# wolearyc/ramannoodle

Hardware: NVIDIA B200
Metric: md_frames_per_s (higher is better)
Workload: dtype f64

## Files before the change

include/ramannoodle_b200_debug.h:

```cpp
#ifndef RAMANNOODLE_B200_DEBUG_H
#define RAMANNOODLE_B200_DEBUG_H

#include "ramannoodle_b200.h"

#ifdef __cplusplus
extern "C" {
#endif

void rn_debug_force_generic_affine(int on);
void rn_debug_set_affine_config(int mt, int stages);
void rn_debug_set_dense_config(int version, int variant);
int64_t rn_debug_phase_tiles(int64_t num_frames, int64_t first_frame, int64_t stripe, int phase, int64_t* tiles,
                             int64_t capacity);
void rn_debug_set_dense_split(int mode);
void rn_debug_set_sweep_fused(int on);
void rn_debug_set_sweep_min_run(int run);
int rn_debug_fft_forward(rn_spectrum_plan* plan, const double* d_in, double* d_out, void* stream);
int rn_debug_fft_convolve(rn_spectrum_plan* plan, const double* d_in, double* d_out, void* stream);

#ifdef __cplusplus
}
#endif

#endif
```

ramannoodle_b200/_lib.py:

```python
from __future__ import annotations

import ctypes
import os

from .exceptions import NativeLibraryError

_HERE = os.path.dirname(os.path.abspath(__file__))
LIB_PATH = os.path.join(_HERE, "libramannoodle_b200.so")

c_double_p = ctypes.POINTER(ctypes.c_double)
c_int32_p = ctypes.POINTER(ctypes.c_int32)
c_int64_p = ctypes.POINTER(ctypes.c_int64)

RN_MODEL_DEFAULT = 0
RN_MODEL_FORCE_DENSE = 1

PROTOTYPES = {
    "rn_last_error": (ctypes.c_char_p, []),
    "rn_device_info": (ctypes.c_int, [ctypes.c_int] + [ctypes.POINTER(ctypes.c_int)] * 4),
    "rn_model_create": (ctypes.c_int, [ctypes.c_void_p, ctypes.c_int64, ctypes.c_void_p, ctypes.c_void_p,
                                       ctypes.c_int64, ctypes.c_void_p, ctypes.c_void_p, ctypes.c_void_p,
                                       ctypes.c_void_p, ctypes.c_void_p, ctypes.c_void_p, ctypes.c_void_p,
                                       ctypes.c_int, ctypes.c_int, ctypes.POINTER(ctypes.c_void_p)]),
    "rn_model_destroy": (ctypes.c_int, [ctypes.c_void_p]),
    "rn_model_info": (ctypes.c_int, [ctypes.c_void_p, c_int64_p]),
    "rn_calc_polarizabilities": (ctypes.c_int, [ctypes.c_void_p, ctypes.c_void_p, ctypes.c_int64,
                                                ctypes.c_void_p, ctypes.c_void_p]),
    "rn_get_polarizability": (ctypes.c_int, [ctypes.c_void_p, ctypes.c_void_p, ctypes.c_int64,
                                             ctypes.c_void_p, ctypes.c_void_p]),
    "rn_calc_polarizabilities_host": (ctypes.c_int, [ctypes.c_void_p, ctypes.c_void_p, ctypes.c_int64,
                                                     ctypes.c_void_p, ctypes.c_void_p, ctypes.c_int64]),
    "rn_calc_polarizabilities_multi": (ctypes.c_int, [ctypes.c_void_p, ctypes.c_void_p, ctypes.c_int64,
                                                      ctypes.c_void_p, ctypes.c_int, ctypes.c_void_p]),
    "rn_calc_polarizabilities_host_multi": (ctypes.c_int, [ctypes.c_void_p, ctypes.c_void_p, ctypes.c_int64,
                                                           ctypes.c_void_p, ctypes.c_int, ctypes.c_int64,
                                                           ctypes.c_void_p]),
    "rn_calc_polarizabilities_routed": (ctypes.c_int, [ctypes.c_void_p, ctypes.c_void_p, ctypes.c_int64,
                                                       ctypes.c_void_p, ctypes.c_void_p, ctypes.c_int, ctypes.c_int64,
                                                       ctypes.c_int64, ctypes.c_int64, ctypes.c_void_p]),
    "rn_routed_phases_supported": (ctypes.c_int, [ctypes.c_void_p, ctypes.c_void_p, ctypes.c_int64, ctypes.c_int64,
                                                  ctypes.c_int64]),
    "rn_calc_polarizabilities_routed_phase": (ctypes.c_int, [ctypes.c_void_p, ctypes.c_void_p, ctypes.c_int64,
                                                             ctypes.c_void_p, ctypes.c_void_p, ctypes.c_int,
                                                             ctypes.c_int64, ctypes.c_int64, ctypes.c_int64,
                                                             ctypes.c_int64, ctypes.c_int, ctypes.c_void_p]),
    "rn_calc_polarizabilities_host_routed": (ctypes.c_int, [ctypes.c_void_p, ctypes.c_void_p, ctypes.c_int64,
                                                            ctypes.c_void_p, ctypes.c_void_p, ctypes.c_int,
                                                            ctypes.c_int64, ctypes.c_int64, ctypes.c_int64,
                                                            ctypes.c_int64, ctypes.c_void_p]),
    "rn_apply_pbc": (ctypes.c_int, [ctypes.c_void_p, ctypes.c_void_p, ctypes.c_int64, ctypes.c_void_p]),
    "rn_spectrum_plan_create": (ctypes.c_int, [ctypes.c_int64, ctypes.c_int, ctypes.POINTER(ctypes.c_void_p)]),
    "rn_spectrum_plan_destroy": (ctypes.c_int, [ctypes.c_void_p]),
    "rn_spectrum_num_points": (ctypes.c_int64, [ctypes.c_int64]),
    "rn_md_spectrum": (ctypes.c_int, [ctypes.c_void_p, ctypes.c_void_p, ctypes.c_double, ctypes.c_int,
                                      ctypes.c_double, ctypes.c_int, ctypes.c_double, ctypes.c_void_p,
                                      ctypes.c_void_p, ctypes.c_void_p]),
    "rn_spectrum_plan_create_dist": (ctypes.c_int, [ctypes.c_int64, ctypes.c_int, ctypes.c_int, ctypes.c_int,
                                                    ctypes.POINTER(ctypes.c_void_p)]),
    "rn_spectrum_plan_info": (ctypes.c_int, [ctypes.c_void_p, c_int64_p]),
    "rn_spectrum_dist_sizes": (ctypes.c_int, [ctypes.c_void_p, c_int64_p, c_int64_p, c_int64_p]),
    "rn_spectrum_dist_route": (ctypes.c_int, [ctypes.c_void_p, c_int64_p, c_int64_p]),
    "rn_spectrum_dist_stripe": (ctypes.c_int, [ctypes.c_void_p, c_int64_p]),
    "rn_spectrum_dist_pack": (ctypes.c_int, [ctypes.c_void_p, ctypes.c_void_p, ctypes.c_void_p, ctypes.c_void_p,
                                             ctypes.c_int, ctypes.c_int, ctypes.c_int, ctypes.c_void_p]),
    "rn_spectrum_dist_transform": (ctypes.c_int, [ctypes.c_void_p, ctypes.c_void_p, ctypes.c_void_p, ctypes.c_int,
                                                  ctypes.c_void_p]),
    "rn_spectrum_dist_final": (ctypes.c_int, [ctypes.c_void_p, ctypes.c_void_p, ctypes.c_void_p, ctypes.c_void_p,
                                              ctypes.c_int, ctypes.c_double, ctypes.c_int, ctypes.c_double,
                                              ctypes.c_int, ctypes.c_double, ctypes.c_void_p, ctypes.c_void_p]),
    "rn_spectrum_dist_finish": (ctypes.c_int, [ctypes.c_void_p, ctypes.c_void_p, ctypes.c_double, ctypes.c_void_p,
                                               ctypes.c_void_p, ctypes.c_void_p]),
    "rn_signal_spectrum": (ctypes.c_int, [ctypes.c_void_p, ctypes.c_void_p, ctypes.c_double, ctypes.c_void_p,
                                          ctypes.c_void_p, ctypes.c_void_p]),
    "rn_convolve_workspace_size": (ctypes.c_size_t, [ctypes.c_int64, ctypes.c_int64]),
    "rn_convolve_spectrum": (ctypes.c_int, [ctypes.c_void_p, ctypes.c_void_p, ctypes.c_int64, ctypes.c_int,
                                            ctypes.c_double, ctypes.c_void_p, ctypes.c_int64, ctypes.c_void_p,
                                            ctypes.c_void_p, ctypes.c_void_p]),
    "rn_calc_polarizabilities_sweep": (ctypes.c_int, [ctypes.c_void_p, ctypes.c_int, ctypes.c_void_p, ctypes.c_int64,
                                                      ctypes.c_void_p, ctypes.c_void_p]),
    "rn_calc_polarizabilities_host_sweep": (ctypes.c_int, [ctypes.c_void_p, ctypes.c_int, ctypes.c_void_p,
                                                           ctypes.c_int64, ctypes.c_void_p, ctypes.c_int64]),
    "rn_calc_polarizabilities_sweep_routed": (ctypes.c_int, [ctypes.c_void_p, ctypes.c_int, ctypes.c_void_p,
                                                             ctypes.c_int64, ctypes.c_void_p, ctypes.c_void_p,
                                                             ctypes.c_int, ctypes.c_int64, ctypes.c_int64,
                                                             ctypes.c_int64, ctypes.c_void_p]),
    "rn_calc_polarizabilities_host_sweep_routed": (ctypes.c_int, [ctypes.c_void_p, ctypes.c_int, ctypes.c_void_p,
                                                                  ctypes.c_int64, ctypes.c_void_p, ctypes.c_void_p,
                                                                  ctypes.c_int, ctypes.c_int64, ctypes.c_int64,
                                                                  ctypes.c_int64, ctypes.c_int64, ctypes.c_void_p]),
    "rn_xdatcar_scan": (ctypes.c_int, [ctypes.c_char_p, c_int64_p, c_int64_p, ctypes.c_void_p]),
    "rn_xdatcar_read": (ctypes.c_int, [ctypes.c_char_p, ctypes.c_void_p, ctypes.c_int64, ctypes.c_int64,
                                       ctypes.c_int, ctypes.c_int]),
    "rn_outcar_scan": (ctypes.c_int, [ctypes.c_char_p, c_int64_p, c_int64_p, ctypes.c_void_p, ctypes.c_void_p]),
    "rn_outcar_read": (ctypes.c_int, [ctypes.c_char_p, ctypes.c_void_p, ctypes.c_int64, ctypes.c_int64,
                                      ctypes.c_void_p, ctypes.c_int, ctypes.c_int]),
    "rn_vasprun_scan": (ctypes.c_int, [ctypes.c_char_p, c_int64_p, c_int64_p, c_double_p]),
    "rn_vasprun_read": (ctypes.c_int, [ctypes.c_char_p, ctypes.c_void_p, ctypes.c_int64, ctypes.c_int64,
                                       ctypes.c_int, ctypes.c_int]),
    "rn_host_apply_pbc": (ctypes.c_int, [ctypes.c_void_p, ctypes.c_void_p, ctypes.c_int64, ctypes.c_int]),
    "rn_host_register": (ctypes.c_int, [ctypes.c_void_p, ctypes.c_size_t]),
    "rn_host_unregister": (ctypes.c_int, [ctypes.c_void_p]),
    "rn_bspline_to_pp": (ctypes.c_int, [ctypes.c_void_p, ctypes.c_int, ctypes.c_void_p, ctypes.c_int,
                                        ctypes.c_void_p, ctypes.c_void_p, ctypes.c_void_p]),
    "rn_launch_count": (ctypes.c_int64, []),
}

DEBUG_PROTOTYPES = {
    "rn_debug_force_generic_affine": (None, [ctypes.c_int]),
    "rn_debug_set_affine_config": (None, [ctypes.c_int, ctypes.c_int]),
    "rn_debug_set_dense_config": (None, [ctypes.c_int, ctypes.c_int]),
    "rn_debug_phase_tiles": (ctypes.c_int64, [ctypes.c_int64, ctypes.c_int64, ctypes.c_int64, ctypes.c_int, c_int64_p,
                                              ctypes.c_int64]),
    "rn_debug_set_dense_split": (None, [ctypes.c_int]),
    "rn_debug_set_sweep_fused": (None, [ctypes.c_int]),
    "rn_debug_set_sweep_min_run": (None, [ctypes.c_int]),
    "rn_debug_fft_forward": (ctypes.c_int, [ctypes.c_void_p, ctypes.c_void_p, ctypes.c_void_p, ctypes.c_void_p]),
    "rn_debug_fft_convolve": (ctypes.c_int, [ctypes.c_void_p, ctypes.c_void_p, ctypes.c_void_p, ctypes.c_void_p]),
}

_lib = None


def lib() -> ctypes.CDLL:
    global _lib
    if _lib is None:
        if not os.path.exists(LIB_PATH):
            raise NativeLibraryError(
                f"{LIB_PATH} not found — build it with `python -m ramannoodle_b200._build` "
                "(there is no CPU fallback)")
        try:
            handle = ctypes.CDLL(LIB_PATH)
        except OSError as exc:
            raise NativeLibraryError(f"cannot load {LIB_PATH}: {exc}") from exc
        for name, (restype, argtypes) in PROTOTYPES.items():
            try:
                fn = getattr(handle, name)
            except AttributeError as exc:
                raise NativeLibraryError(f"{LIB_PATH} does not export {name}") from exc
            fn.restype = restype
            fn.argtypes = argtypes
        for name, (restype, argtypes) in DEBUG_PROTOTYPES.items():
            fn = getattr(handle, name)
            fn.restype = restype
            fn.argtypes = argtypes
        _lib = handle
    return _lib


def last_error() -> str:
    return lib().rn_last_error().decode("utf-8", "replace")


def check(status: int, what: str) -> None:
    if status == 0:
        return
    message = last_error()
    if status == -1:
        raise ValueError(f"{what}: {message}")
    if status == -4:
        raise MemoryError(f"{what}: {message}")
    raise NativeLibraryError(f"{what} failed ({status}): {message}")


def require_device(device: int = 0) -> dict:
    rt = ctypes.c_int()
    count = ctypes.c_int()
    cc = ctypes.c_int()
    sms = ctypes.c_int()
    status = lib().rn_device_info(device, ctypes.byref(rt), ctypes.byref(count), ctypes.byref(cc), ctypes.byref(sms))
    if status != 0:
        raise NativeLibraryError(f"no usable CUDA device {device}: {last_error()} (there is no CPU fallback)")
    if cc.value // 10 != 10:
        raise NativeLibraryError(f"device {device} is sm_{cc.value}; ramannoodle_b200 is built for sm_100a only")
    return {"runtime": rt.value, "devices": count.value, "compute_capability": cc.value, "sm_count": sms.value}


def launch_count() -> int:
    return int(lib().rn_launch_count())
```

ramannoodle_b200/csrc/rn_device.cuh:

```cuda
#pragma once

#include "rn_common.cuh"

namespace rn {

struct Alpha0 {
    double v[9];
};

__device__ __forceinline__ double wrap_disp(double pos, double ref) {
    const double d = pos - ref;
    return d - ceil(d - 0.5);
}

__device__ __forceinline__ double wrap_disp_fast(double pos, double ref) {
    const double d = pos - ref;
    const unsigned mag = (unsigned)__double2hiint(d) & 0x7fffffffu;
    if (mag < 0x3fe00000u) return d;
    return d - ceil(d - 0.5);
}

__device__ __forceinline__ void dmma884(double& c0, double& c1, double a, double b) {
    asm("mma.sync.aligned.m8n8k4.row.col.f64.f64.f64.f64 {%0,%1}, {%2}, {%3}, {%0,%1};"
        : "+d"(c0), "+d"(c1)
        : "d"(a), "d"(b));
}

__device__ __forceinline__ uint32_t smem_u32(const void* p) { return (uint32_t)__cvta_generic_to_shared(p); }

__device__ __forceinline__ void cp_async_16(uint32_t dst, const void* src, int src_bytes) {
    asm volatile("cp.async.cg.shared.global [%0], [%1], 16, %2;" ::"r"(dst), "l"(src), "r"(src_bytes) : "memory");
}
__device__ __forceinline__ void cp_async_8(uint32_t dst, const void* src, int src_bytes) {
    asm volatile("cp.async.ca.shared.global [%0], [%1], 8, %2;" ::"r"(dst), "l"(src), "r"(src_bytes) : "memory");
}
__device__ __forceinline__ void cp_async_commit() { asm volatile("cp.async.commit_group;" ::: "memory"); }
template <int N>
__device__ __forceinline__ void cp_async_wait() {
    asm volatile("cp.async.wait_group %0;" ::"n"(N) : "memory");
}

__device__ __forceinline__ void mbar_init(uint32_t bar, uint32_t count) {
    asm volatile("mbarrier.init.shared::cta.b64 [%0], %1;" ::"r"(bar), "r"(count) : "memory");
}
__device__ __forceinline__ void mbar_arrive_expect_tx(uint32_t bar, uint32_t bytes) {
    asm volatile("mbarrier.arrive.expect_tx.shared::cta.b64 _, [%0], %1;" ::"r"(bar), "r"(bytes) : "memory");
}
__device__ __forceinline__ void mbar_wait(uint32_t bar, uint32_t parity) {
    asm volatile(
        "{\n"
        ".reg .pred p;\n"
        "WAIT_%=:\n"
        "mbarrier.try_wait.parity.shared::cta.b64 p, [%0], %1;\n"
        "@p bra DONE_%=;\n"
        "bra WAIT_%=;\n"
        "DONE_%=:\n"
        "}\n" ::"r"(bar),
        "r"(parity)
        : "memory");
}
__device__ __forceinline__ void tma_bulk_g2s(uint32_t dst, const void* src, uint32_t bytes, uint32_t bar) {
    asm volatile("cp.async.bulk.shared::cluster.global.mbarrier::complete_tx::bytes [%0], [%1], %2, [%3];" ::"r"(dst),
                 "l"(src), "r"(bytes), "r"(bar)
                 : "memory");
}

}
```

ramannoodle_b200/csrc/rn_polarizability.cu:

```cuda
#include "rn_device.cuh"

namespace rn {

template <bool WRAP>
__global__ void __launch_bounds__(256) affine_generic_kernel(const double* __restrict__ in,
                                                             const double* __restrict__ ref,
                                                             const double* __restrict__ G, int64_t frame_begin,
                                                             int64_t frame_end, int K, Alpha0 a0,
                                                             double* __restrict__ alpha) {
    const int lane = threadIdx.x & 31;
    const int g = lane >> 2, t = lane & 3;
    const int64_t warps = (int64_t)gridDim.x * (blockDim.x >> 5);
    const int64_t groups = (frame_end - frame_begin + 7) / 8;
    for (int64_t grp = (int64_t)blockIdx.x * (blockDim.x >> 5) + (threadIdx.x >> 5); grp < groups; grp += warps) {
        const int64_t frame = frame_begin + grp * 8 + g;
        const bool valid = frame < frame_end;
        const double* row = in + (valid ? frame : frame_begin) * (int64_t)K;
        double c0 = 0, c1 = 0, d0 = 0, d1 = 0;
        for (int e0 = 0; e0 < K; e0 += 4) {
            const int e = e0 + t;
            double a = 0, b = 0, b2 = 0;
            if (e < K) {
                if (valid) {
                    a = __ldg(row + e);
// ... 64 lines not shown

    if (threadIdx.x == 0) {
        for (int s = 0; s < STAGES; s++) mbar_init(full0 + 8 * s, 1);
        asm volatile("fence.mbarrier_init.release.cluster;" ::: "memory");
        asm volatile("fence.proxy.async;" ::: "memory");
        for (int s = 0; s < STAGES; s++) {
            const int64_t tile = blockIdx.x + (int64_t)s * gridDim.x;
            if (tile < num_tiles) issue_tile(tile, s);
        }
    }
    for (int e = threadIdx.x; e < slack; e += blockDim.x) {
        tab_ref[e] = WRAP ? __ldg(ref + e) : 0.0;
        tab_g9[e] = __ldg(G + (int64_t)e * 9 + 8);
    }
    __syncthreads();

    const int g = lane >> 2, t = lane & 3;
    const int kbase = warp * 8 * KP + 2 * t;
    double b8[KP][2];
    uint32_t validmask = 0;
#pragma unroll
    for (int p = 0; p < KP; p++) {
#pragma unroll
        for (int h = 0; h < 2; h++) {
            const int e = kbase + 8 * p + h;
            b8[p][h] = __ldg(G + (int64_t)e * 9 + g);
            if (e < K) validmask |= 1u << (2 * p + h);
        }
    }
    const double* my_ref = tab_ref + kbase;
    const double* my_g9 = tab_g9 + kbase;
    const int rowoff = g * row_stride + kbase;
    double* myred = red + ((size_t)warp * ROWS + g) * kRedStride;

    int64_t i = 0;
    int64_t pending_row0 = -1;
    TileCursor here, ahead;
    if (SELECT) {
        cursor_set(sel, blockIdx.x, here);
        cursor_set(sel, blockIdx.x + (int64_t)STAGES * gridDim.x, ahead);
    }
    for (int64_t tile = blockIdx.x; tile < num_tiles; tile += gridDim.x, i++) {
        const int s = (int)(i % STAGES);
        const int64_t tile_row0 = (SELECT ? cursor_tile(sel, here) : tile) * ROWS;
        const bool stage_rows = peers_bulk && (tile_row0 + ROWS <= num_frames);
        mbar_wait(full0 + 8 * s, (uint32_t)(i / STAGES) & 1);
        const double* base = stages + (size_t)s * stage_doubles + rowoff;
        double c0[MT][2], c1[MT][2], a9[MT][2];
#pragma unroll
        for (int m = 0; m < MT; m++)
#pragma unroll
            for (int h = 0; h < 2; h++) c0[m][h] = c1[m][h] = a9[m][h] = 0.0;
#pragma unroll
        for (int p = 0; p < KP; p++) {
            const double2 g9 = *reinterpret_cast<const double2*>(my_g9 + 8 * p);
            double2 rf = make_double2(0.0, 0.0);
            if (WRAP) rf = *reinterpret_cast<const double2*>(my_ref + 8 * p);
#pragma unroll
            for (int m = 0; m < MT; m++) {
                const double2 v = *reinterpret_cast<const double2*>(base + (size_t)m * 8 * row_stride + 8 * p);
                double a_lo = v.x, a_hi = v.y;
                if (WRAP) {
                    a_lo = wrap_disp(a_lo, rf.x);
                    a_hi = wrap_disp(a_hi, rf.y);
                }
                a_lo = (validmask >> (2 * p)) & 1u ? a_lo : 0.0;
                a_hi = (validmask >> (2 * p + 1)) & 1u ? a_hi : 0.0;
                dmma884(c0[m][0], c1[m][0], a_lo, b8[p][0]);
                a9[m][0] = fma(a_lo, g9.x, a9[m][0]);
                dmma884(c0[m][1], c1[m][1], a_hi, b8[p][1]);
                a9[m][1] = fma(a_hi, g9.y, a9[m][1]);
            }
        }
        double* slot = myred + (size_t)(i & 1) * RED;
#pragma unroll
        for (int m = 0; m < MT; m++) {
            double a9s = a9[m][0] + a9[m][1];
            a9s += __shfl_xor_sync(0xffffffffu, a9s, 1);
            a9s += __shfl_xor_sync(0xffffffffu, a9s, 2);
            *reinterpret_cast<double2*>(slot + (size_t)m * 8 * kRedStride + 2 * t) =
                make_double2(c0[m][0] + c0[m][1], c1[m][0] + c1[m][1]);
            if (t == 0) slot[(size_t)m * 8 * kRedStride + 8] = a9s;
        }
        __syncthreads();
        if (peers_bulk && threadIdx.x == 32 && pending_row0 >= 0) {
            const uint32_t src = smem_u32(outbuf + (size_t)((i - 1) & 1) * ROWS * 9);
            const uint32_t mask = alpha_peer_mask(peers, pending_row0, ROWS);
            const int64_t off = alpha_peer_offset(peers, pending_row0);
            for (int p = 0; p < peers.count; p++)
                if (((mask >> p) & 1u) && peers.ptr[p])
                    asm volatile("cp.async.bulk.global.shared::cta.bulk_group [%0], [%1], %2;" ::"l"(peers.ptr[p] + off),
                                 "r"(src), "r"((uint32_t)(ROWS * 72))
                                 : "memory");
            asm volatile("cp.async.bulk.commit_group;" ::: "memory");
        }
        {
            const int64_t next = tile + (int64_t)STAGES * gridDim.x;
            if (next < num_tiles && lane == 0) {
                const int64_t frame0 = (SELECT ? cursor_tile(sel, ahead) : next) * ROWS;
                const int rows = (int)min((int64_t)ROWS, num_frames - frame0);
                if (warp == 0) mbar_arrive_expect_tx(full0 + 8 * s, row_bytes * rows);
                const uint32_t dst0 = smem_u32(stages + (size_t)s * stage_doubles);
                const double* src0 = in + frame0 * (int64_t)K;
                for (int r = warp; r < rows; r += kAffineWarps)
                    tma_bulk_g2s(dst0 + (uint32_t)(r * row_stride) * 8u, src0 + (int64_t)r * K, row_bytes,
                                 full0 + 8 * s);
            }
        }
        if (threadIdx.x < 9 * ROWS) {
            const int f = threadIdx.x / 9, q = threadIdx.x % 9;
            const double* r = red + (size_t)(i & 1) * RED + (size_t)f * kRedStride + q;
            double sum = 0;
#pragma unroll
            for (int w = 0; w < kAffineWarps; w++) sum += r[(size_t)w * ROWS * kRedStride];
            const int64_t frame = tile_row0 + f;
            const double value = sum + a0.v[q];
            if (frame < num_frames) alpha[frame * 9 + q] = value;
            if (stage_rows) {
                outbuf[(size_t)(i & 1) * ROWS * 9 + threadIdx.x] = value;
                asm volatile("fence.proxy.async.shared::cta;" ::: "memory");
            } else if (frame < num_frames) {
                const uint32_t mask = alpha_peer_mask(peers, frame, 1);
                const int64_t off = alpha_peer_offset(peers, frame);
                for (int p = 0; p < peers.count; p++)
                    if (((mask >> p) & 1u) && peers.ptr[p]) peers.ptr[p][off + q] = value;
            }
        }
        if (peers_bulk && threadIdx.x == 32) {
            asm volatile("cp.async.bulk.wait_group.read 0;" ::: "memory");
        }
        pending_row0 = stage_rows ? tile_row0 : -1;
        if (SELECT) {
            cursor_advance(sel, gridDim.x, here);
            cursor_advance(sel, gridDim.x, ahead);
        }
    }
    if (peers_bulk) {
        __syncthreads();
        if (threadIdx.x == 32 && pending_row0 >= 0) {
            const uint32_t src = smem_u32(outbuf + (size_t)((i - 1) & 1) * ROWS * 9);
            const uint32_t mask = alpha_peer_mask(peers, pending_row0, ROWS);
            const int64_t off = alpha_peer_offset(peers, pending_row0);
            for (int p = 0; p < peers.count; p++)
                if (((mask >> p) & 1u) && peers.ptr[p])
                    asm volatile("cp.async.bulk.global.shared::cta.bulk_group [%0], [%1], %2;" ::"l"(peers.ptr[p] + off),
                                 "r"(src), "r"((uint32_t)(ROWS * 72))
                                 : "memory");
            asm volatile("cp.async.bulk.commit_group;" ::: "memory");
        }
        if (threadIdx.x == 32) asm volatile("cp.async.bulk.wait_group 0;" ::: "memory");
    }
}

static std::atomic<int> g_affine_mt{0};

template <int KP, int MT, int STAGES, bool WRAP>
static int launch_affine_tma_cfg(const rn_model* m, const double* d_in, int64_t frames, double* d_alpha, Alpha0 a0,
                                 cudaStream_t stream, const AlphaPeers& peers) {
    const int K = (int)m->dim;
    const AffineSmemLayout L = affine_layout(K, KP, MT, STAGES);
    if (L.bytes > 227 * 1024) return 1;
    const TileSelect sel = peers.sel_stripe > 0 ? phase_tiles(peers.first_frame, frames, peers.sel_stripe, peers.sel_phase, 8 * MT)
                                                : all_tiles();
    const int64_t tiles = sel.period ? sel.count : (frames + 8 * MT - 1) / (8 * MT);
    if (tiles == 0) return RN_OK;
    const double* ref = WRAP ? m->d_ref_wrapped : m->d_zero_ref;
    const double* G = WRAP ? m->d_g_frac : m->d_g_cart;
    auto kern = sel.period ? affine_tma_kernel<KP, MT, STAGES, WRAP, true> : affine_tma_kernel<KP, MT, STAGES, WRAP, false>;
    RN_CUDA(cudaFuncSetAttribute(kern, cudaFuncAttributeMaxDynamicSharedMemorySize, (int)L.bytes));
    int ctas_per_sm = 1;
    RN_CUDA(cudaOccupancyMaxActiveBlocksPerMultiprocessor(&ctas_per_sm, kern, kAffineWarps * 32, L.bytes));
    if (ctas_per_sm < 1) return 1;
    const int grid = (int)std::min<int64_t>(tiles, (int64_t)m->sm_count * ctas_per_sm);
    int peers_bulk = peers.count > 0 ? 1 : 0;
    for (int p = 0; p < peers.count; p++)
        if (peers.ptr[p] && reinterpret_cast<uintptr_t>(peers.ptr[p]) % 16 != 0) peers_bulk = 0;
    if (peers.log2_period >= 0 && (peers.first_frame * 72) % 16 != 0) peers_bulk = 0;
    kern<<<grid, kAffineWarps * 32, L.bytes, stream>>>(d_in, ref, G, frames, K, L.row_stride, L.stage_doubles, a0,
                                                       d_alpha, peers, peers_bulk, sel);
    RN_LAUNCHED();
    RN_CUDA(cudaGetLastError());
    return RN_OK;
}

template <int KP, bool WRAP>
static int launch_affine_tma_kp(const rn_model* m, const double* d_in, int64_t frames, double* d_alpha, Alpha0 a0,
                                cudaStream_t stream, const AlphaPeers& peers) {
    int mt = g_affine_mt.load(std::memory_order_relaxed);
    if (mt == 0) mt = (KP >= 8) ? 2 : 1;
    int rc = 1;
    if (mt == 2) rc = launch_affine_tma_cfg<KP, 2, 2, WRAP>(m, d_in, frames, d_alpha, a0, stream, peers);
    if (rc == 1) rc = launch_affine_tma_cfg<KP, 1, 2, WRAP>(m, d_in, frames, d_alpha, a0, stream, peers);
    return rc;
}

template <bool WRAP>
static int launch_affine_tma(const rn_model* m, const double* d_in, int64_t frames, double* d_alpha, Alpha0 a0,
                             cudaStream_t stream, const AlphaPeers& peers) {
    switch (m->affine_kp) {
#define RN_AFFINE_CASE(KP) \
    case KP: return launch_affine_tma_kp<KP, WRAP>(m, d_in, frames, d_alpha, a0, stream, peers);
        RN_AFFINE_CASE(1)
        RN_AFFINE_CASE(2)
        RN_AFFINE_CASE(3)
        RN_AFFINE_CASE(4)
        RN_AFFINE_CASE(5)
        RN_AFFINE_CASE(6)
        RN_AFFINE_CASE(7)
        RN_AFFINE_CASE(8)
        RN_AFFINE_CASE(9)
        RN_AFFINE_CASE(10)
        RN_AFFINE_CASE(11)
        RN_AFFINE_CASE(12)
#undef RN_AFFINE_CASE
        default:
            set_error("affine TMA kernel not compiled for KP=%d", m->affine_kp);
            return RN_ERR_UNSUPPORTED;
    }
}

template <bool WRAP>
static int launch_affine_generic(const rn_model* m, const double* d_in, int64_t begin, int64_t end, double* d_alpha,
                                 Alpha0 a0, cudaStream_t stream) {
    if (end <= begin) return RN_OK;
    const int64_t groups = (end - begin + 7) / 8;
    const int grid = (int)std::min<int64_t>((groups + 7) / 8, (int64_t)m->sm_count * 8);
    affine_generic_kernel<WRAP><<<grid, 256, 0, stream>>>(d_in, WRAP ? m->d_ref_wrapped : m->d_zero_ref,
                                                          WRAP ? m->d_g_frac : m->d_g_cart, begin, end, (int)m->dim, a0,
                                                          d_alpha);
    RN_LAUNCHED();
    RN_CUDA(cudaGetLastError());
    return RN_OK;
}

static std::atomic<bool> g_force_generic_affine{false};

int launch_affine(const rn_model* m, const double* d_in, bool wrap, int64_t num_frames, double* d_alpha,
                  cudaStream_t stream, const AlphaPeers* peers, bool* peers_done) {
    Alpha0 a0;
    for (int q = 0; q < 9; q++) a0.v[q] = m->alpha0[q];
    const int K = (int)m->dim;
    const bool aligned = (reinterpret_cast<uintptr_t>(d_in) % 16) == 0 && (K % 2 == 0);
    int64_t tma_frames = 0;
    if (m->affine_kp > 0 && aligned && !g_force_generic_affine.load(std::memory_order_relaxed)) {
        tma_frames = num_frames;
    }
    int rc = RN_OK;
    AlphaPeers fused = no_peers();
    if (peers) fused = *peers;
    if (tma_frames > 0) {
        rc = wrap ? launch_affine_tma<true>(m, d_in, tma_frames, d_alpha, a0, stream, fused)
                  : launch_affine_tma<false>(m, d_in, tma_frames, d_alpha, a0, stream, fused);
        if (rc == 1) {
            tma_frames = 0;
            rc = RN_OK;
        }
        if (rc != RN_OK) return rc;
    }
    if (fused.sel_stripe > 0 && tma_frames != num_frames) {
        set_error("a frame selection (pipelined multi-GPU schedule) needs the TMA affine kernel");
        return RN_ERR_UNSUPPORTED;
    }
    if (peers_done) *peers_done = (tma_frames == num_frames);
    if (tma_frames < num_frames) {
        rc = wrap ? launch_affine_generic<true>(m, d_in, tma_frames, num_frames, d_alpha, a0, stream)
                  : launch_affine_generic<false>(m, d_in, tma_frames, num_frames, d_alpha, a0, stream);
    }
    return rc;
}

__global__ void fill_alpha0_kernel(int64_t count, Alpha0 a0, double* __restrict__ alpha) {
    for (int64_t i = blockIdx.x * (int64_t)blockDim.x + threadIdx.x; i < count; i += (int64_t)gridDim.x * blockDim.x)
        alpha[i] = a0.v[i % 9];
}

int launch_fill_alpha0(const rn_model* m, int64_t num_frames, double* d_alpha, cudaStream_t stream) {
    if (num_frames == 0) return RN_OK;
    Alpha0 a0;
    for (int q = 0; q < 9; q++) a0.v[q] = m->alpha0[q];
    const int64_t count = num_frames * 9;
    const int grid = (int)std::min<int64_t>((count + 255) / 256, (int64_t)m->sm_count * 8);
    fill_alpha0_kernel<<<grid, 256, 0, stream>>>(count, a0, d_alpha);
    RN_LAUNCHED();
    RN_CUDA(cudaGetLastError());
    return RN_OK;
}

constexpr int kFT = 128;
constexpr int kJT = 64;
constexpr int kKC = 16;
constexpr int kRS = 20;
constexpr int kDStages = 3;

template <int DEG, bool WRAP, bool ALIGN16>
__global__ void __launch_bounds__(256, 1)
    dense_kernel(const double* __restrict__ in, const double* __restrict__ ref, const double* __restrict__ V,
                 const int32_t* __restrict__ piece_off, const double* __restrict__ breaks,
                 const double* __restrict__ pieces, int64_t num_frames, int K, int Kv, int Jpad, int accumulate,
                 Alpha0 a0, double* __restrict__ alpha) {
    extern __shared__ __align__(128) unsigned char smem_raw[];
    double* As = reinterpret_cast<double*>(smem_raw);
    double* Bs = As + (size_t)kDStages * kFT * kRS;
    constexpr int REC = 1 + 9 * (DEG + 1);

    const int warp = threadIdx.x >> 5, lane = threadIdx.x & 31;
    const int g = lane >> 2, t = lane & 3;
    const int chunks = Kv / kKC;
    const int jtiles = Jpad / kJT;
    const int64_t total = (int64_t)jtiles * chunks;
    const int64_t num_tiles = (num_frames + kFT - 1) / kFT;

    for (int64_t tile = blockIdx.x; tile < num_tiles; tile += gridDim.x) {
        const int64_t frame0 = tile * kFT;

        auto issue = [&](int64_t it) {
            if (it < total) {
                const int jt = (int)(it / chunks), kc = (int)(it % chunks);
                const int st = (int)(it % kDStages);
                double* a_dst = As + (size_t)st * kFT * kRS;
                double* b_dst = Bs + (size_t)st * kJT * kRS;
                if (ALIGN16) {
#pragma unroll
                    for (int r = 0; r < (kFT * 8) / 256; r++) {
                        const int idx = threadIdx.x + 256 * r;
                        const int row = idx >> 3, seg = idx & 7;
                        const int col = kc * kKC + seg * 2;
                        const int64_t frame = frame0 + row;
                        int bytes = 0;
                        if (frame < num_frames && col < K) bytes = min(16, (K - col) * 8);
                        const double* src = in + (bytes ? frame * (int64_t)K + col : 0);
                        cp_async_16(smem_u32(a_dst + row * kRS + seg * 2), src, bytes);
                    }
                } else {
#pragma unroll
                    for (int r = 0; r < (kFT * 16) / 256; r++) {
                        const int idx = threadIdx.x + 256 * r;
                        const int row = idx >> 4, seg = idx & 15;
                        const int col = kc * kKC + seg;
                        const int64_t frame = frame0 + row;
                        const int bytes = (frame < num_frames && col < K) ? 8 : 0;
                        const double* src = in + (bytes ? frame * (int64_t)K + col : 0);
                        cp_async_8(smem_u32(a_dst + row * kRS + seg), src, bytes);
                    }
// ... 146 lines not shown
        default:
            set_error("dense kernel not compiled for spline degree %d", m->dense_degree);
            return RN_ERR_UNSUPPORTED;
    }
}

}

using namespace rn;

static int eval_common(const rn_model* model, const double* d_in, bool wrap, int64_t num_frames, double* d_alpha,
                       void* stream, const AlphaPeers* peers = nullptr) {
    RN_CHECK_ARG(model != nullptr, "model is null");
    RN_CHECK_ARG(num_frames >= 0, "num_frames must be non-negative");
    if (num_frames == 0) return RN_OK;
    RN_CHECK_ARG(d_in && d_alpha, "null device pointer");
    DeviceGuard guard(model->device);
    if (!guard.ok) {
        set_error("cudaSetDevice(%d) failed", model->device);
        return RN_ERR_CUDA;
    }
    cudaStream_t s = static_cast<cudaStream_t>(stream);
    if (peers && peers->count == 0) peers = nullptr;
    int rc = RN_OK;
    bool peers_done = false;
    if (model->num_dofs == 0) {
        rc = launch_fill_alpha0(model, num_frames, d_alpha, s);
    } else {
        const bool run_affine = model->num_linear > 0;
        const bool run_dense = model->num_dense > 0;
        if (run_affine) {
            rc = launch_affine(model, d_in, wrap, num_frames, d_alpha, s, run_dense ? nullptr : peers, &peers_done);
            if (rc != RN_OK) return rc;
        }
        if (run_dense) rc = launch_dense(model, d_in, wrap, run_affine, num_frames, d_alpha, s, peers, &peers_done);
    }
    if (rc != RN_OK) return rc;
    if (peers && !peers_done) {
        for (int p = 0; p < peers->count; p++)
            if (peers->ptr[p])
                RN_CUDA(cudaMemcpyAsync(peers->ptr[p] + alpha_peer_offset(*peers, 0), d_alpha,
                                        sizeof(double) * 9 * num_frames, cudaMemcpyDeviceToDevice, s));
    }
    return RN_OK;
}

static int make_peers(double* const* d_alpha_outputs, int num_outputs, AlphaPeers* peers) {
    RN_CHECK_ARG(d_alpha_outputs != nullptr && num_outputs >= 1 && num_outputs <= 8,
                 "between 1 and 8 output pointers are required");
    *peers = no_peers();
    peers->count = num_outputs - 1;
    for (int i = 0; i < num_outputs; i++) RN_CHECK_ARG(d_alpha_outputs[i] != nullptr, "null output pointer");
    for (int i = 1; i < num_outputs; i++) peers->ptr[i - 1] = d_alpha_outputs[i];
    return RN_OK;
}

extern "C" int rn_calc_polarizabilities_multi(const rn_model* model, const double* d_positions, int64_t num_frames,
                                              double* const* d_alpha_outputs, int num_outputs, void* stream) {
    AlphaPeers peers;
    int rc = make_peers(d_alpha_outputs, num_outputs, &peers);
    if (rc != RN_OK) return rc;
    return eval_common(model, d_positions, true, num_frames, d_alpha_outputs[0], stream, &peers);
}

int rn::make_routed_peers(double* const* peer_series, int world, int64_t first_frame, int64_t period, int64_t width,
                          AlphaPeers* peers) {
    RN_CHECK_ARG(peer_series != nullptr && world >= 1 && world <= 8, "between 1 and 8 ranks");
    RN_CHECK_ARG(first_frame >= 0, "first_frame must be non-negative");
    RN_CHECK_ARG(period > 0 && (period & (period - 1)) == 0 && width >= 32 && (width & (width - 1)) == 0 &&
                     width <= period && period / width <= world,
                 "period and width must be powers of two with width >= 32 and period / width <= world");
    *peers = no_peers();
    peers->count = world;
    for (int r = 0; r < world; r++) peers->ptr[r] = peer_series[r];
    peers->log2_period = 0;
    while (((int64_t)1 << peers->log2_period) < period) peers->log2_period++;
    peers->log2_width = 0;
    while (((int64_t)1 << peers->log2_width) < width) peers->log2_width++;
    peers->first_frame = first_frame;
    return RN_OK;
}

int rn::eval_with_peers(const rn_model* model, const double* d_positions, int64_t num_frames, double* d_alpha,
                        cudaStream_t stream, const AlphaPeers& peers) {
    return eval_common(model, d_positions, true, num_frames, d_alpha, stream, &peers);
}

extern "C" int rn_calc_polarizabilities_routed(const rn_model* model, const double* d_positions, int64_t num_frames,
                                               double* d_alpha, double* const* peer_series, int world,
                                               int64_t first_frame, int64_t period, int64_t width, void* stream) {
    AlphaPeers peers;
    int rc = make_routed_peers(peer_series, world, first_frame, period, width, &peers);
    if (rc != RN_OK) return rc;
    return eval_common(model, d_positions, true, num_frames, d_alpha, stream, &peers);
}

static bool routed_phases_ok(const rn_model* model, const double* d_positions, int64_t num_frames, int64_t first_frame,
                             int64_t stripe) {
    if (!model || model->num_dofs == 0 || model->num_dense > 0 || model->num_linear == 0 || model->affine_kp <= 0) return false;
    if (g_force_generic_affine.load(std::memory_order_relaxed)) return false;
    if (reinterpret_cast<uintptr_t>(d_positions) % 16 != 0 || model->dim % 2 != 0) return false;
    return stripe >= 1024 && (stripe & (stripe - 1)) == 0 && num_frames % 16 == 0 && first_frame % 16 == 0 &&
           num_frames >= 16;
}

extern "C" int rn_routed_phases_supported(const rn_model* model, const double* d_positions, int64_t num_frames,
                                          int64_t first_frame, int64_t stripe) {
    return routed_phases_ok(model, d_positions, num_frames, first_frame, stripe) ? 1 : 0;
}

extern "C" int rn_calc_polarizabilities_routed_phase(const rn_model* model, const double* d_positions,
                                                     int64_t num_frames, double* d_alpha, double* const* peer_series,
                                                     int world, int64_t first_frame, int64_t period, int64_t width,
                                                     int64_t stripe, int phase, void* stream) {
    RN_CHECK_ARG(phase == 0 || phase == 1, "phase must be 0 or 1");
    if (!routed_phases_ok(model, d_positions, num_frames, first_frame, stripe)) {
        set_error("this model / trajectory block cannot be evaluated in phases (rn_routed_phases_supported)");
        return RN_ERR_UNSUPPORTED;
    }
    AlphaPeers peers;
    int rc = make_routed_peers(peer_series, world, first_frame, period, width, &peers);
    if (rc != RN_OK) return rc;
    peers.sel_stripe = stripe;
    peers.sel_phase = phase;
    return eval_common(model, d_positions, true, num_frames, d_alpha, stream, &peers);
}

extern "C" int rn_calc_polarizabilities(const rn_model* model, const double* d_positions, int64_t num_frames,
                                        double* d_alpha, void* stream) {
    return eval_common(model, d_positions, true, num_frames, d_alpha, stream);
}

extern "C" int rn_get_polarizability(const rn_model* model, const double* d_cart_displacements, int64_t num_frames,
                                     double* d_alpha, void* stream) {
    return eval_common(model, d_cart_displacements, false, num_frames, d_alpha, stream);
}

extern "C" int64_t rn_debug_phase_tiles(int64_t num_frames, int64_t first_frame, int64_t stripe, int phase,
                                        int64_t* tiles, int64_t capacity) {
    const TileSelect sel = phase_tiles(first_frame, num_frames, stripe, phase, 16);
    for (int64_t start = 0; start < 2; start++) {
        TileCursor c;
        cursor_set(sel, start, c);
        for (int64_t j = start; j < sel.count; j += 2, cursor_advance(sel, 2, c)) {
            if (cursor_tile(sel, c) != select_tile(sel, j)) return -1;
            if (j < capacity) tiles[j] = cursor_tile(sel, c);
        }
    }
    return sel.count;
}

extern "C" void rn_debug_force_generic_affine(int on) { rn::g_force_generic_affine.store(on != 0, std::memory_order_relaxed); }
extern "C" void rn_debug_set_affine_config(int mt, int stages) {
    (void)stages;
    rn::g_affine_mt.store(mt, std::memory_order_relaxed);
}

__global__ void apply_pbc_kernel(const double* __restrict__ in, double* __restrict__ out, int64_t count) {
    for (int64_t i = blockIdx.x * (int64_t)blockDim.x + threadIdx.x; i < count; i += (int64_t)gridDim.x * blockDim.x) {
        const double p = in[i];
        out[i] = p - floor(p);
    }
}

extern "C" int rn_apply_pbc(const double* d_in, double* d_out, int64_t count, void* stream) {
    RN_CHECK_ARG(count >= 0, "count must be non-negative");
    if (count == 0) return RN_OK;
    RN_CHECK_ARG(d_in && d_out, "null device pointer");
    const int grid = (int)std::min<int64_t>((count + 255) / 256, 148 * 16);
    apply_pbc_kernel<<<grid, 256, 0, static_cast<cudaStream_t>(stream)>>>(d_in, d_out, count);
    RN_LAUNCHED();
    RN_CUDA(cudaGetLastError());
    return RN_OK;
}
```

Baseline: 1.011 billion.

## Add warp-specialized streaming affine kernel with TMA producer and reducer warps

Adds a new affine polarizability kernel that uses a dedicated producer warp issuing bulk TMA row loads into an mbarrier-managed ring of slots. A dedicated reducer warp sums the per-warp partials and writes alpha, with bulk stores to peer buffers. Eight compute warps run DMMA on the loaded tiles, and the reduction is double-buffered. This is meant to overlap loading, computing and output writing in a persistent pipeline, in place of the staged TMA kernel. In exchange it brings in a more complex barrier protocol and higher shared-memory use, and it keeps a fallback to the old kernel plus a debug switch to select it.

```diff
diff --git a/include/ramannoodle_b200_debug.h b/include/ramannoodle_b200_debug.h
--- a/include/ramannoodle_b200_debug.h
+++ b/include/ramannoodle_b200_debug.h
@@ -9,6 +9,7 @@
 
 void rn_debug_force_generic_affine(int on);
 void rn_debug_set_affine_config(int mt, int stages);
+void rn_debug_set_affine_version(int version);
 void rn_debug_set_dense_config(int version, int variant);
 int64_t rn_debug_phase_tiles(int64_t num_frames, int64_t first_frame, int64_t stripe, int phase, int64_t* tiles,
                              int64_t capacity);
diff --git a/ramannoodle_b200/_lib.py b/ramannoodle_b200/_lib.py
--- a/ramannoodle_b200/_lib.py
+++ b/ramannoodle_b200/_lib.py
@@ -108,6 +108,7 @@
 DEBUG_PROTOTYPES = {
     "rn_debug_force_generic_affine": (None, [ctypes.c_int]),
     "rn_debug_set_affine_config": (None, [ctypes.c_int, ctypes.c_int]),
+    "rn_debug_set_affine_version": (None, [ctypes.c_int]),
     "rn_debug_set_dense_config": (None, [ctypes.c_int, ctypes.c_int]),
     "rn_debug_phase_tiles": (ctypes.c_int64, [ctypes.c_int64, ctypes.c_int64, ctypes.c_int64, ctypes.c_int, c_int64_p,
                                               ctypes.c_int64]),
diff --git a/ramannoodle_b200/csrc/rn_device.cuh b/ramannoodle_b200/csrc/rn_device.cuh
--- a/ramannoodle_b200/csrc/rn_device.cuh
+++ b/ramannoodle_b200/csrc/rn_device.cuh
@@ -46,6 +46,9 @@
 __device__ __forceinline__ void mbar_arrive_expect_tx(uint32_t bar, uint32_t bytes) {
     asm volatile("mbarrier.arrive.expect_tx.shared::cta.b64 _, [%0], %1;" ::"r"(bar), "r"(bytes) : "memory");
 }
+__device__ __forceinline__ void mbar_arrive(uint32_t bar) {
+    asm volatile("mbarrier.arrive.shared::cta.b64 _, [%0];" ::"r"(bar) : "memory");
+}
 __device__ __forceinline__ void mbar_wait(uint32_t bar, uint32_t parity) {
     asm volatile(
         "{\n"
diff --git a/ramannoodle_b200/csrc/rn_polarizability.cu b/ramannoodle_b200/csrc/rn_polarizability.cu
--- a/ramannoodle_b200/csrc/rn_polarizability.cu
+++ b/ramannoodle_b200/csrc/rn_polarizability.cu
@@ -240,7 +240,250 @@
     }
 }
 
+constexpr int kStreamWarps = 8;
+constexpr int kStreamThreads = (kStreamWarps + 2) * 32;
+constexpr int kStreamRed = 2;
+constexpr int kStreamMaxKP = 9;
+constexpr int stream_ctas(int kp, int mt) { return (kp <= 6 && mt == 1) ? 2 : 1; }
+
+static size_t stream_smem_bytes(int row_stride, int kp, int mt, int slots) {
+    const int slack = kStreamWarps * 8 * kp;
+    return (size_t)(slots * 8 * row_stride + slack) * 8 + (size_t)kStreamRed * kStreamWarps * 8 * mt * kRedStride * 8 +
+           (size_t)2 * slack * 8 + (size_t)8 * mt * 9 * 8 + (size_t)(2 * slots + 2 * kStreamRed) * 8;
+}
+
+template <int KP, int MT, bool WRAP>
+__global__ void __launch_bounds__(kStreamThreads, stream_ctas(KP, MT))
+    affine_stream_kernel(const double* __restrict__ in, const double* __restrict__ ref, const double* __restrict__ G,
+                         int64_t num_frames, int K, int row_stride, int slots, Alpha0 a0, double* __restrict__ alpha,
+                         AlphaPeers peers, int peers_bulk) {
+    extern __shared__ __align__(128) unsigned char smem_raw[];
+    constexpr int ROWS = 8 * MT;
+    constexpr int RED = kStreamWarps * ROWS * kRedStride;
+    const int slot_doubles = 8 * row_stride;
+    const int slack = kStreamWarps * 8 * KP;
+    double* ring = reinterpret_cast<double*>(smem_raw);
+    double* red = ring + (size_t)slots * slot_doubles + slack;
+    double* tab_ref = red + kStreamRed * RED;
+    double* tab_g9 = tab_ref + slack;
+    double* outbuf = tab_g9 + slack;
+    uint64_t* bars = reinterpret_cast<uint64_t*>(outbuf + ROWS * 9);
+    const uint32_t full0 = smem_u32(bars), empty0 = full0 + 8 * slots;
+    const uint32_t redfull0 = empty0 + 8 * slots, redfree0 = redfull0 + 8 * kStreamRed;
+
+    const int warp = threadIdx.x >> 5, lane = threadIdx.x & 31;
+    const int64_t num_tiles = (num_frames + ROWS - 1) / ROWS;
+    const int64_t my_tiles = blockIdx.x < num_tiles ? (num_tiles - 1 - blockIdx.x) / gridDim.x + 1 : 0;
+    const int64_t total_q = my_tiles * MT;
+    const uint32_t row_bytes = (uint32_t)K * 8u;
+
+    if (threadIdx.x == 0) {
+        for (int s = 0; s < slots; s++) {
+            mbar_init(full0 + 8 * s, 1);
+            mbar_init(empty0 + 8 * s, kStreamWarps);
+        }
+        for (int r = 0; r < kStreamRed; r++) {
+            mbar_init(redfull0 + 8 * r, kStreamWarps);
+            mbar_init(redfree0 + 8 * r, 1);
+        }
+        asm volatile("fence.mbarrier_init.release.cluster;" ::: "memory");
+        asm volatile("fence.proxy.async;" ::: "memory");
+    }
+    for (int e = threadIdx.x; e < slack; e += blockDim.x) {
+        tab_ref[e] = WRAP ? __ldg(ref + e) : 0.0;
+        tab_g9[e] = __ldg(G + (int64_t)e * 9 + 8);
+    }
+    __syncthreads();
+
+    if (warp == kStreamWarps) {
+        int s = 0;
+        uint32_t ph = 0;
+        for (int64_t q = 0; q < total_q; q++) {
+            mbar_wait(empty0 + 8 * s, ph ^ 1u);
+            const int64_t frame0 = (blockIdx.x + (q / MT) * (int64_t)gridDim.x) * ROWS + (q % MT) * 8;
+            const int rows = (int)max((int64_t)0, min((int64_t)8, num_frames - frame0));
+            if (lane == 0) mbar_arrive_expect_tx(full0 + 8 * s, row_bytes * rows);
+            __syncwarp();
+            if (lane < rows)
+                tma_bulk_g2s(smem_u32(ring + (size_t)s * slot_doubles + (size_t)lane * row_stride),
+                             in + (frame0 + lane) * (int64_t)K, row_bytes, full0 + 8 * s);
+            if (++s == slots) {
+                s = 0;
+                ph ^= 1u;
+            }
+        }
+        return;
+    }
+    if (warp == kStreamWarps + 1) {
+        for (int64_t i = 0; i < my_tiles; i++) {
+            const int r = (int)(i & 1);
+            mbar_wait(redfull0 + 8 * r, (uint32_t)(i >> 1) & 1u);
+            const int64_t tile_row0 = (blockIdx.x + i * (int64_t)gridDim.x) * ROWS;
+            const bool stage_rows = peers_bulk && (tile_row0 + ROWS <= num_frames);
+            if (stage_rows) {
+                if (lane == 0) asm volatile("cp.async.bulk.wait_group.read 0;" ::: "memory");
+                __syncwarp();
+            }
+            const double* part = red + (size_t)r * RED;
+            for (int idx = lane; idx < 9 * ROWS; idx += 32) {
+                const int f = idx / 9, q = idx - 9 * f;
+                const double* p = part + (size_t)f * kRedStride + q;
+                double sum = 0;
+#pragma unroll
+                for (int w = 0; w < kStreamWarps; w++) sum += p[(size_t)w * ROWS * kRedStride];
+                const int64_t frame = tile_row0 + f;
+                const double value = sum + a0.v[q];
+                if (frame < num_frames) alpha[frame * 9 + q] = value;
+                if (stage_rows) {
+                    outbuf[idx] = value;
+                } else if (frame < num_frames) {
+                    const uint32_t mask = alpha_peer_mask(peers, frame, 1);
+                    const int64_t off = alpha_peer_offset(peers, frame);
+                    for (int p = 0; p < peers.count; p++)
+                        if (((mask >> p) & 1u) && peers.ptr[p]) peers.ptr[p][off + q] = value;
+                }
+            }
+            if (stage_rows) asm volatile("fence.proxy.async.shared::cta;" ::: "memory");
+            __syncwarp();
+            if (lane == 0) {
+                mbar_arrive(redfree0 + 8 * r);
+                if (stage_rows) {
+                    const uint32_t src = smem_u32(outbuf);
+                    const uint32_t mask = alpha_peer_mask(peers, tile_row0, ROWS);
+                    const int64_t off = alpha_peer_offset(peers, tile_row0);
+                    for (int p = 0; p < peers.count; p++)
+                        if (((mask >> p) & 1u) && peers.ptr[p])
+                            asm volatile("cp.async.bulk.global.shared::cta.bulk_group [%0], [%1], %2;" ::"l"(peers.ptr[p] + off),
+                                         "r"(src), "r"((uint32_t)(ROWS * 72))
+                                         : "memory");
+                    asm volatile("cp.async.bulk.commit_group;" ::: "memory");
+                }
+            }
+        }
+        if (peers_bulk && lane == 0) asm volatile("cp.async.bulk.wait_group 0;" ::: "memory");
+        return;
+    }
+
+    const int g = lane >> 2, t = lane & 3;
+    const int kbase = warp * 8 * KP + 2 * t;
+    double b8[KP][2];
+    uint32_t validmask = 0;
+#pragma unroll
+    for (int p = 0; p < KP; p++) {
+#pragma unroll
+        for (int h = 0; h < 2; h++) {
+            const int e = kbase + 8 * p + h;
+            b8[p][h] = __ldg(G + (int64_t)e * 9 + g);
+            if (e < K) validmask |= 1u << (2 * p + h);
+        }
+    }
+    const double* my_ref = tab_ref + kbase;
+    const double* my_g9 = tab_g9 + kbase;
+    const int rowoff = g * row_stride + kbase;
+    double* myred = red + ((size_t)warp * ROWS + g) * kRedStride;
+
+    int cs = 0;
+    uint32_t cph = 0;
+    for (int64_t i = 0; i < my_tiles; i++) {
+        int sl[MT];
+        const double* base[MT];
+#pragma unroll
+        for (int m = 0; m < MT; m++) {
+            sl[m] = cs;
+            mbar_wait(full0 + 8 * cs, cph);
+            base[m] = ring + (size_t)cs * slot_doubles + rowoff;
+            if (++cs == slots) {
+                cs = 0;
+                cph ^= 1;
+            }
+        }
+        double c0[MT][2], c1[MT][2], a9[MT][2];
+#pragma unroll
+        for (int m = 0; m < MT; m++)
+#pragma unroll
+            for (int h = 0; h < 2; h++) c0[m][h] = c1[m][h] = a9[m][h] = 0.0;
+#pragma unroll
+        for (int p = 0; p < KP; p++) {
+            const double2 g9 = *reinterpret_cast<const double2*>(my_g9 + 8 * p);
+            double2 rf = make_double2(0.0, 0.0);
+            if (WRAP) rf = *reinterpret_cast<const double2*>(my_ref + 8 * p);
+#pragma unroll
+            for (int m = 0; m < MT; m++) {
+                const double2 v = *reinterpret_cast<const double2*>(base[m] + 8 * p);
+                double a_lo = v.x, a_hi = v.y;
+                if (WRAP) {
+                    a_lo = wrap_disp(a_lo, rf.x);
+                    a_hi = wrap_disp(a_hi, rf.y);
+                }
+                a_lo = (validmask >> (2 * p)) & 1u ? a_lo : 0.0;
+                a_hi = (validmask >> (2 * p + 1)) & 1u ? a_hi : 0.0;
+                dmma884(c0[m][0], c1[m][0], a_lo, b8[p][0]);
+                a9[m][0] = fma(a_lo, g9.x, a9[m][0]);
+                dmma884(c0[m][1], c1[m][1], a_hi, b8[p][1]);
+                a9[m][1] = fma(a_hi, g9.y, a9[m][1]);
+            }
+        }
+        __syncwarp();
+        if (lane == 0) {
+#pragma unroll
+            for (int m = 0; m < MT; m++) mbar_arrive(empty0 + 8 * sl[m]);
+        }
+        const int r = (int)(i & 1);
+        mbar_wait(redfree0 + 8 * r, ((uint32_t)(i >> 1) & 1u) ^ 1u);
+        double* slot = myred + (size_t)r * RED;
+#pragma unroll
+        for (int m = 0; m < MT; m++) {
+            double a9s = a9[m][0] + a9[m][1];
+            a9s += __shfl_xor_sync(0xffffffffu, a9s, 1);
+            a9s += __shfl_xor_sync(0xffffffffu, a9s, 2);
+            *reinterpret_cast<double2*>(slot + (size_t)m * 8 * kRedStride + 2 * t) =
+                make_double2(c0[m][0] + c0[m][1], c1[m][0] + c1[m][1]);
+            if (t == 0) slot[(size_t)m * 8 * kRedStride + 8] = a9s;
+        }
+        __syncwarp();
+        if (lane == 0) mbar_arrive(redfull0 + 8 * r);
+    }
+}
+
 static std::atomic<int> g_affine_mt{0};
+static std::atomic<int> g_affine_slots{0};
+static std::atomic<int> g_affine_version{0};
+
+static int peers_bulk_ok(const AlphaPeers& peers) {
+    int peers_bulk = peers.count > 0 ? 1 : 0;
+    for (int p = 0; p < peers.count; p++)
+        if (peers.ptr[p] && reinterpret_cast<uintptr_t>(peers.ptr[p]) % 16 != 0) peers_bulk = 0;
+    if (peers.log2_period >= 0 && (peers.first_frame * 72) % 16 != 0) peers_bulk = 0;
+    return peers_bulk;
+}
+
+template <int KP, int MT, bool WRAP>
+static int launch_affine_stream_cfg(const rn_model* m, const double* d_in, int64_t frames, double* d_alpha, Alpha0 a0,
+                                    cudaStream_t stream, const AlphaPeers& peers) {
+    const int K = (int)m->dim;
+    const int row_stride = K + (8 - K % 16 + 16) % 16;
+    int slots = g_affine_slots.load(std::memory_order_relaxed);
+    if (slots <= 0) slots = stream_ctas(KP, MT) == 2 ? 2 : 4;
+    slots = std::max(slots, std::max(2, MT));
+    const size_t bytes = stream_smem_bytes(row_stride, KP, MT, slots);
+    if (bytes > 227 * 1024) return 1;
+    const int64_t tiles = (frames + 8 * MT - 1) / (8 * MT);
+    if (tiles == 0) return RN_OK;
+    const double* ref = WRAP ? m->d_ref_wrapped : m->d_zero_ref;
+    const double* G = WRAP ? m->d_g_frac : m->d_g_cart;
+    auto kern = affine_stream_kernel<KP, MT, WRAP>;
+    constexpr int threads = kStreamThreads;
+    RN_CUDA(cudaFuncSetAttribute(kern, cudaFuncAttributeMaxDynamicSharedMemorySize, (int)bytes));
+    int ctas_per_sm = 1;
+    RN_CUDA(cudaOccupancyMaxActiveBlocksPerMultiprocessor(&ctas_per_sm, kern, threads, bytes));
+    if (ctas_per_sm < 1) return 1;
+    const int grid = (int)std::min<int64_t>(tiles, (int64_t)m->sm_count * ctas_per_sm);
+    kern<<<grid, threads, bytes, stream>>>(d_in, ref, G, frames, K, row_stride, slots, a0, d_alpha, peers,
+                                           peers_bulk_ok(peers));
+    RN_LAUNCHED();
+    RN_CUDA(cudaGetLastError());
+    return RN_OK;
+}
 
 template <int KP, int MT, int STAGES, bool WRAP>
 static int launch_affine_tma_cfg(const rn_model* m, const double* d_in, int64_t frames, double* d_alpha, Alpha0 a0,
@@ -260,12 +503,8 @@
     RN_CUDA(cudaOccupancyMaxActiveBlocksPerMultiprocessor(&ctas_per_sm, kern, kAffineWarps * 32, L.bytes));
     if (ctas_per_sm < 1) return 1;
     const int grid = (int)std::min<int64_t>(tiles, (int64_t)m->sm_count * ctas_per_sm);
-    int peers_bulk = peers.count > 0 ? 1 : 0;
-    for (int p = 0; p < peers.count; p++)
-        if (peers.ptr[p] && reinterpret_cast<uintptr_t>(peers.ptr[p]) % 16 != 0) peers_bulk = 0;
-    if (peers.log2_period >= 0 && (peers.first_frame * 72) % 16 != 0) peers_bulk = 0;
     kern<<<grid, kAffineWarps * 32, L.bytes, stream>>>(d_in, ref, G, frames, K, L.row_stride, L.stage_doubles, a0,
-                                                       d_alpha, peers, peers_bulk, sel);
+                                                       d_alpha, peers, peers_bulk_ok(peers), sel);
     RN_LAUNCHED();
     RN_CUDA(cudaGetLastError());
     return RN_OK;
@@ -277,6 +516,13 @@
     int mt = g_affine_mt.load(std::memory_order_relaxed);
     if (mt == 0) mt = (KP >= 8) ? 2 : 1;
     int rc = 1;
+    if constexpr (KP <= kStreamMaxKP) {
+        if (peers.sel_stripe == 0 && g_affine_version.load(std::memory_order_relaxed) != 1) {
+            if (mt == 2) rc = launch_affine_stream_cfg<KP, 2, WRAP>(m, d_in, frames, d_alpha, a0, stream, peers);
+            if (rc == 1) rc = launch_affine_stream_cfg<KP, 1, WRAP>(m, d_in, frames, d_alpha, a0, stream, peers);
+            if (rc != 1) return rc;
+        }
+    }
     if (mt == 2) rc = launch_affine_tma_cfg<KP, 2, 2, WRAP>(m, d_in, frames, d_alpha, a0, stream, peers);
     if (rc == 1) rc = launch_affine_tma_cfg<KP, 1, 2, WRAP>(m, d_in, frames, d_alpha, a0, stream, peers);
     return rc;
@@ -729,8 +975,11 @@
 
 extern "C" void rn_debug_force_generic_affine(int on) { rn::g_force_generic_affine.store(on != 0, std::memory_order_relaxed); }
 extern "C" void rn_debug_set_affine_config(int mt, int stages) {
-    (void)stages;
     rn::g_affine_mt.store(mt, std::memory_order_relaxed);
+    rn::g_affine_slots.store(stages, std::memory_order_relaxed);
+}
+extern "C" void rn_debug_set_affine_version(int version) {
+    rn::g_affine_version.store(version, std::memory_order_relaxed);
 }
 
 __global__ void apply_pbc_kernel(const double* __restrict__ in, double* __restrict__ out, int64_t count) {
```

Result: faster. 1.098 billion, median of 6 (+8.6%).
